# yanielc/medical-vision-textural-bias

Hardware: AMD Instinct MI355X
Metric: BraTS 4ch 240^3 vols/sec filtered+train-step @1/2/4/8 GPU; filter HBM GB/s (higher is better)
Workload: dtype f32

## Files before the change

### medical-vision-textural-bias_amd/csrc/conv_up.hip

```cpp
#include <hip/hip_runtime.h>

#include <cstdlib>
#include <type_traits>

#include "conv_host.h"
#include "split_bf16.h"
#include "texbias.h"

namespace {

typedef float f2v __attribute__((ext_vector_type(2)));
typedef float f32x4 __attribute__((ext_vector_type(4)));
typedef const __attribute__((address_space(4))) float* cfloat_p;
typedef const __attribute__((address_space(4))) f2v* cf2v_p;

template <int B, int N, class F>
__device__ __forceinline__ void static_for(F&& f) {
  if constexpr (B < N) {
    f(std::integral_constant<int, B>{});
    static_for<B + 1, N>(f);
  }
}

struct S2Args {
// ... 868 lines not shown
  for (int j = 0; j < NL; ++j) {
    const int i = tid + 256 * j;
    const int c = i / per_c, r2 = i - c * per_c, r = r2 / W4, q = r2 - r * W4;
    const int yi = y0 + r;
    lof[j] = i < total ? c * RX + r * PX + 4 * q : Wi;
    gof[j] = (i < total && yi < Hi) ? yi * Wi + 4 * q : -1;
    gch[j] = i < total ? c : 0;
  }
  float4 rg[NL];
  auto load = [&](int zi) {
    const bool in = zi < Di;
    const float* src = xb + (int64_t)(in ? zi : 0) * plane;
#pragma unroll
    for (int j = 0; j < NL; ++j) {
      const bool ok = in && gof[j] >= 0;
      rg[j] = *reinterpret_cast<const float4*>(src + gch[j] * cstride + (ok ? gof[j] : 0));
    }
  };
  auto store = [&](int zi) {
    float* d = ring + (zi & 1) * SS;
    const bool in = zi < Di;
#pragma unroll
    for (int j = 0; j < NL; ++j)
      *reinterpret_cast<float4*>(d + lof[j]) = (in && gof[j] >= 0) ? rg[j] : make_float4(0.f, 0.f, 0.f, 0.f);
  };
  float bm[4];
#pragma unroll
  for (int r = 0; r < 4; ++r) bm[r] = a.bias ? a.bias[4 * ks + r] : 0.f;
  __syncthreads();
  load(z0);
  store(z0);
  load(z0 + 1);
  store(z0 + 1);
  __builtin_amdgcn_s_waitcnt(0x0F70);
  __syncthreads();
  const int npos = YB * Wi, ntile = (npos + 15) / 16;
  const int64_t oplane = 4 * plane, orow = 2 * Wi;
  float* yb0 = a.y + (int64_t)n * 16 * (2 * Di) * oplane;
  auto sums = [&](int z, int t0, int pb) {
    const float* pr = part + pb * 4 * 8 * 256;
    for (int k = w; k < 4 * HT; k += 4) {
      const int hq = k >> 2, pz = (k >> 1) & 1, py = k & 1, q0 = pz * 4 + py * 2;
      const int pq = 16 * (t0 + hq) + li, yq = pq / Wi, xq = pq - yq * Wi;
      const bool okp = t0 + hq < ntile && pq < npos && y0 + yq < Hi;
#pragma unroll
      for (int r = 0; r < 4; ++r) {
        const int m = 4 * ks + r, e = m * 16 + li;
        float v0 = bm[r], v1 = bm[r];
#pragma unroll
        for (int v = 0; v < G; ++v) {
          v0 += pr[((hq * G + v) * 8 + q0) * 256 + e];
          v1 += pr[((hq * G + v) * 8 + q0 + 1) * 256 + e];
        }
        if (okp)
          *reinterpret_cast<float2*>(yb0 + ((int64_t)m * (2 * Di) + 2 * z + pz) * oplane +
                                     (int64_t)(2 * (y0 + yq) + py) * orow + 2 * xq) = make_float2(v0, v1);
      }
    }
  };
  int buf = 0;
  for (int z = z0; z < z1; ++z) {
    if (z + 1 < z1) load(z + 2);
    const float* sz[2] = {ring + (z & 1) * SS, ring + ((z + 1) & 1) * SS};
    for (int t0 = 0; t0 < ntile; t0 += HT) {
      const int tI = t0 + h;
      const int p = 16 * tI + li, pc = p < npos ? p : npos - 1;
      const int yy = pc / Wi, xx = pc - yy * Wi;
      const int bl = (16 * g + ks) * RX + yy * PX + xx;
      f32x4 acc[8];
#pragma unroll
      for (int q = 0; q < 8; ++q) acc[q] = f32x4{0.f, 0.f, 0.f, 0.f};
#pragma unroll
      for (int tz = 0; tz < 3; ++tz)
#pragma unroll
        for (int ty = 0; ty < 3; ++ty)
#pragma unroll
          for (int tx = 0; tx < 3; ++tx) {
            const int t = tz * 9 + ty * 3 + tx;
            const int par = (tz != 1) * 4 + (ty != 1) * 2 + (tx != 1);
            const float* s = sz[tz == 0] + bl + (ty == 0) * PX + (tx == 0);
#pragma unroll
            for (int cq = 0; cq < 4; ++cq)
              acc[par] = __builtin_amdgcn_mfma_f32_16x16x4f32(af[4 * t + cq], s[4 * cq * RX], acc[par], 0, 0, 0);
          }
      float* pw = part + (buf * 4 + w) * 8 * 256;
#pragma unroll
      for (int q = 0; q < 8; ++q)
#pragma unroll
        for (int r = 0; r < 4; ++r) pw[q * 256 + (4 * ks + r) * 16 + li] = acc[q][r];
      __syncthreads();
      if (t0 > 0) sums(z, t0 - HT, buf ^ 1);
      buf ^= 1;
    }
    store(z + 2);
    sums(z, ((ntile - 1) / HT) * HT, buf ^ 1);
    __syncthreads();
  }
}
}

int tb_convT3d_mfma64_f32(const float* x, const float* W, const float* bias, float* y, int N, int Di, int Hi, int Wi,
                          void* stream) {
  return tb_convT3d_mfma_f32(x, W, bias, y, N, 64, Di, Hi, Wi, stream);
}

int tb_convT3d_mfma_f32(const float* x, const float* W, const float* bias, float* y, int N, int Cin, int Di, int Hi,
                        int Wi, void* stream) {
  if (!x || !W || !y || N < 1 || Di < 1 || Hi < 1 || Wi < 1) return TB_ERR_INVALID_ARG;
  if (Cin != 32 && Cin != 64) return TB_ERR_UNSUPPORTED_SIZE;
  if (Wi % 4 != 0 || Wi > 64 || (reinterpret_cast<uintptr_t>(x) & 15) != 0 || (reinterpret_cast<uintptr_t>(y) & 7) != 0)
    return TB_ERR_UNSUPPORTED_SIZE;
  constexpr int YB = 2;
  T64Args a{};
  a.x = x, a.W = W, a.bias = bias, a.y = y, a.Di = Di, a.Hi = Hi, a.Wi = Wi;
  a.PX = Wi + 4;
  a.RX = (YB + 1) * a.PX;
  while ((a.RX & 31) != 16) ++a.RX;
  a.nyb = (Hi + YB - 1) / YB;
  const size_t lds = (size_t)4 * (2 * Cin * a.RX + 2 * 4 * 8 * 256);
  if (lds > 163840) return TB_ERR_UNSUPPORTED_SIZE;
  a.zlen = tb::zseg(Di, N * a.nyb, 1, 1);
  a.ZS = (Di + a.zlen - 1) / a.zlen;
  const int nl = (Cin * (YB + 1) * (Wi / 4) + 255) / 256;
  void (*kern)(T64Args) = nullptr;
  switch (nl) {
#define TB_NL(k) \
  case k: kern = Cin == 64 ? k_convT_mfma64<4, YB, k> : k_convT_mfma64<2, YB, k>; break;
    TB_NL(1) TB_NL(2) TB_NL(3) TB_NL(4) TB_NL(5) TB_NL(6) TB_NL(7) TB_NL(8) TB_NL(9) TB_NL(10) TB_NL(11) TB_NL(12)
#undef TB_NL
    default: return TB_ERR_UNSUPPORTED_SIZE;
  }
  return tb::launch_lds(kern, dim3((unsigned)(N * a.nyb * a.ZS)), dim3(256), lds,
                        reinterpret_cast<hipStream_t>(stream), a);
}

namespace {
struct S1Args {
  const float* x;
  const float* W;
  const float* bias;
  const float* add;
  float* y;
  int D, H, Wd, YB;
  int ZS, zlen, nyb, MG;
  int PX, RX;
  int flip;
  int64_t addsn;
};

template <int G, int NC, int NL, int NTH, bool ADD = false>
__global__ __launch_bounds__(NTH) void k_conv3d_mfma_s1(S1Args a) {
  constexpr int CIN = 16 * G, MTB = 4 / G, NWG = NTH / 256;
  extern __shared__ __attribute__((aligned(16))) float smem[];
  const int tid = (int)threadIdx.x, lane = tid & 63;
  const int w = __builtin_amdgcn_readfirstlane(tid >> 6);
  const int g = w % G, mt = (w / G) % MTB, h = w / 4;
  const int D = a.D, H = a.H, Wd = a.Wd, YB = a.YB, PX = a.PX, RX = a.RX, SS = CIN * RX;
  const int NR = YB + 2;
  float* ring = smem;
  float* part = smem + 3 * SS;
  float* bsm = part + (NTH / 64) * NC * 256;
  for (int i = tid; i < 3 * SS; i += NTH) ring[i] = 0.f;
  int b = (int)blockIdx.x;
  const int zs = b % a.ZS;
  b /= a.ZS;
  const int mg = b % a.MG;
  b /= a.MG;
  const int yb = b % a.nyb, n = b / a.nyb;
  const int COUT = 16 * MTB * a.MG;
  const int y0 = yb * YB;
  const int z0 = zs * a.zlen, z1 = min(D, z0 + a.zlen);
  const int li = lane & 15, ks = lane >> 4;
  const int m0 = (mg * MTB + mt) * 16;
  if (tid < MTB * 16) bsm[tid] = a.bias ? a.bias[mg * MTB * 16 + tid] : 0.f;
  float af[108];
#pragma unroll
  for (int kk = 0; kk < 108; ++kk) {
    const int c = 16 * g + 4 * (kk & 3) + ks, t = kk >> 2;
    af[kk] = a.flip ? a.W[(c * CIN + m0 + li) * 27 + 26 - t] : a.W[((m0 + li) * CIN + c) * 27 + t];
  }
  const int64_t plane = (int64_t)H * Wd, cstride = (int64_t)D * plane;
  const float* xb = a.x + (int64_t)n * CIN * cstride;
  const int W4 = Wd >> 2, per_c = NR * W4, total = CIN * per_c;
  int gof[NL], lof[NL], gch[NL];
#pragma unroll
  for (int j = 0; j < NL; ++j) {
    const int i = tid + NTH * j;
    const int c = i / per_c, r2 = i - c * per_c, r = r2 / W4, q = r2 - r * W4;
    const int yi = y0 - 1 + r;
    lof[j] = i < total ? c * RX + r * PX + 4 + 4 * q : 0;
    gof[j] = (i < total && yi >= 0 && yi < H) ? yi * Wd + 4 * q : -1;
    gch[j] = i < total ? c : 0;
  }
  float4 rg[NL];
  auto load = [&](int zi) {
    const bool in = zi >= 0 && zi < D;
    const float* src = xb + (int64_t)(in ? zi : 0) * plane;
#pragma unroll
    for (int j = 0; j < NL; ++j) {
      const bool ok = in && gof[j] >= 0;
      rg[j] = *reinterpret_cast<const float4*>(src + gch[j] * cstride + (ok ? gof[j] : 0));
    }
  };
  auto store = [&](int zi) {
    float* d = ring + ((zi + 3) % 3) * SS;
    const bool in = zi >= 0 && zi < D;
#pragma unroll
    for (int j = 0; j < NL; ++j)
      *reinterpret_cast<float4*>(d + lof[j]) = (in && gof[j] >= 0) ? rg[j] : make_float4(0.f, 0.f, 0.f, 0.f);
  };
  __syncthreads();
  load(z0 - 1);
  store(z0 - 1);
  load(z0);
  store(z0);
  load(z0 + 1);
  store(z0 + 1);
  __builtin_amdgcn_s_waitcnt(0x0F70);
  __syncthreads();
  const int npos = YB * Wd;
  float* ybase = a.y + (int64_t)n * COUT * cstride;
  const float* abase = ADD ? a.add + (int64_t)n * (a.addsn ? a.addsn : COUT * cstride) : nullptr;
  constexpr int NK = (MTB * NWG * NC + NTH / 64 - 1) / (NTH / 64);
  int bl[NC];
#pragma unroll
  for (int c = 0; c < NC; ++c) {
    const int p = 16 * (NWG * c + h) + li, pc = p < npos ? p : npos - 1;
    const int yy = pc / Wd, xx = pc - yy * Wd;
    bl[c] = (16 * g + ks) * RX + yy * PX + xx + 3;
  }
  for (int z = z0; z < z1; ++z) {
    if (z + 1 < z1) load(z + 2);
    float av[NK][4];
    if constexpr (ADD) {
#pragma unroll
      for (int kk = 0; kk < NK; ++kk) {
        const int k = w + kk * (NTH / 64);
        if (k >= MTB * NWG * NC) break;
        const int mq = k / (NWG * NC), r2 = k - mq * (NWG * NC), hq = r2 / NC, c = r2 - hq * NC;
        const int p = 16 * (NWG * c + hq) + li, pc = p < npos ? p : npos - 1;
        const int yy = pc / Wd, xx = pc - yy * Wd, yr = min(y0 + yy, H - 1);
        const int mb = (mg * MTB + mq) * 16;
#pragma unroll
        for (int r = 0; r < 4; ++r)
          av[kk][r] = abase[(int64_t)(mb + 4 * ks + r) * cstride + (int64_t)z * plane + (int64_t)yr * Wd + xx];
      }
    }
    const float* sp[3] = {ring + ((z + 2) % 3) * SS, ring + (z % 3) * SS, ring + ((z + 1) % 3) * SS};
    f32x4 acc[NC];
#pragma unroll
    for (int c = 0; c < NC; ++c) acc[c] = f32x4{0.f, 0.f, 0.f, 0.f};
#pragma unroll
    for (int tz = 0; tz < 3; ++tz)
#pragma unroll
      for (int ty = 0; ty < 3; ++ty)
#pragma unroll
        for (int tx = 0; tx < 3; ++tx) {
          const int t = tz * 9 + ty * 3 + tx;
          const float* s = sp[tz] + ty * PX + tx;
#pragma unroll
          for (int cq = 0; cq < 4; ++cq)
#pragma unroll
            for (int c = 0; c < NC; ++c)
              acc[c] = __builtin_amdgcn_mfma_f32_16x16x4f32(af[4 * t + cq], s[bl[c] + 4 * cq * RX], acc[c], 0, 0, 0);
        }
    float* pw = part + w * NC * 256;
#pragma unroll
    for (int c = 0; c < NC; ++c)
#pragma unroll
      for (int r = 0; r < 4; ++r) pw[c * 256 + (4 * ks + r) * 16 + li] = acc[c][r];
    __syncthreads();
    store(z + 2);
    auto combo = [&](int k, int kk) {
      const int mq = k / (NWG * NC), r2 = k - mq * (NWG * NC), hq = r2 / NC, c = r2 - hq * NC;
      const int p = 16 * (NWG * c + hq) + li;
      const int yy = p / Wd, xx = p - yy * Wd;
      const bool ok = p < npos && y0 + yy < H;
      const int mb = (mg * MTB + mq) * 16;
#pragma unroll
      for (int r = 0; r < 4; ++r) {
        const int m = 4 * ks + r;
        float v = bsm[mq * 16 + m];
#pragma unroll
        for (int gg = 0; gg < G; ++gg) v += part[((hq * 4 + mq * G + gg) * NC + c) * 256 + m * 16 + li];
        const int64_t o = (int64_t)(mb + m) * cstride + (int64_t)z * plane + (int64_t)(y0 + yy) * Wd + xx;
        if (ok) ybase[o] = ADD ? v + av[kk][r] : v;
      }
    };
    if constexpr (ADD) {
#pragma unroll
      for (int kk = 0; kk < NK; ++kk) {
        const int k = w + kk * (NTH / 64);
        if (k >= MTB * NWG * NC) break;
        combo(k, kk);
      }
    } else {
      for (int k = w; k < MTB * NWG * NC; k += NTH / 64) combo(k, 0);
    }
    __syncthreads();
  }
}
}

int tb_conv3d_mfma_f32(const float* x, const float* W, const float* bias, float* y, int N, int C, int D, int H, int Wd,
                       void* stream) {
  return tb_conv3d_mfma_add_f32(x, W, bias, nullptr, y, N, C, D, H, Wd, stream);
}

static int mfma_call(const float* x, const float* W, const float* bias, const float* add, float* y, int N, int C, int D,
                     int H, int Wd, int flip, void* stream, int64_t add_sn = 0);

int tb_conv3d_mfma_add_f32(const float* x, const float* W, const float* bias, const float* add, float* y, int N, int C,
                           int D, int H, int Wd, void* stream) {
  return mfma_call(x, W, bias, add, y, N, C, D, H, Wd, 0, stream);
}

int tb_conv3d_mfma_dgrad_f32(const float* gy, const float* W, const float* add, int64_t add_sn, float* dx, int N, int C,
                             int D, int H, int Wd, void* stream) {
  return mfma_call(gy, W, nullptr, add, dx, N, C, D, H, Wd, 1, stream, add_sn);
}

static int mfma_call(const float* x, const float* W, const float* bias, const float* add, float* y, int N, int C, int D,
                     int H, int Wd, int flip, void* stream, int64_t add_sn) {
  if (!x || !W || !y || N < 1 || D < 1 || H < 1 || Wd < 1) return TB_ERR_INVALID_ARG;
  if ((C != 32 && C != 64) || Wd % 4 != 0 || Wd > 64 || (reinterpret_cast<uintptr_t>(x) & 15) != 0)
    return TB_ERR_UNSUPPORTED_SIZE;
  constexpr int NC = 5;
  const int G = C / 16;
  S1Args a{};
  a.x = x, a.W = W, a.bias = bias, a.add = add, a.y = y, a.D = D, a.H = H, a.Wd = Wd;
  a.flip = flip;
  a.addsn = add_sn;
  a.PX = Wd + 8;
  a.MG = G == 2 ? 1 : 4;
  size_t lds = 0;
  int YB = std::max(1, 16 * NC / Wd);
  for (; YB >= 1; --YB) {
    a.RX = (YB + 2) * a.PX;
    while ((a.RX & 31) != 16) ++a.RX;
    lds = (size_t)4 * (3 * C * a.RX + 4 * NC * 256 + 64);
    if (lds <= 163840) break;
  }
  if (YB < 1) return TB_ERR_UNSUPPORTED_SIZE;
  a.YB = YB > H ? H : YB;
  a.nyb = (H + a.YB - 1) / a.YB;
  a.zlen = tb::zseg(D, N * a.nyb * a.MG, 1, 2);
  a.ZS = (D + a.zlen - 1) / a.zlen;
  const int nl = (C * (a.YB + 2) * (Wd / 4) + 255) / 256;
  void (*kern)(S1Args) = nullptr;
#define TB_NL(k)                                                                                      \
  case k:                                                                                             \
    kern = add ? (G == 2 ? k_conv3d_mfma_s1<2, 5, k, 256, true> : k_conv3d_mfma_s1<4, 5, k, 256, true>) \
               : (G == 2 ? k_conv3d_mfma_s1<2, 5, k, 256> : k_conv3d_mfma_s1<4, 5, k, 256>);             \
    break;
  switch (nl) {
    TB_NL(1) TB_NL(2) TB_NL(3) TB_NL(4) TB_NL(5) TB_NL(6) TB_NL(7) TB_NL(8) TB_NL(9) TB_NL(10) TB_NL(11) TB_NL(12)
    default: return TB_ERR_UNSUPPORTED_SIZE;
  }
#undef TB_NL
  return tb::launch_lds(kern, dim3((unsigned)(N * a.nyb * a.MG * a.ZS)), dim3(256), lds,
                        reinterpret_cast<hipStream_t>(stream), a);
}
```

Before: 186.1.

## Add z-streaming split-bf16 MFMA conv kernel with register-resident weights and LDS ring

Adds a new 3D conv kernel for C=32/64 that keeps the split-bf16 weight fragments in registers and streams input z-planes through a 3-slot LDS ring. Input planes are pre-split into three bf16 parts when stored, with the next plane prefetched into registers during compute. Partial sums from the channel groups are reduced through LDS before bias/add and the store. It becomes the default path whenever the plan fits, trading higher register pressure and extra LDS synchronisation for less global reload of the input halo and less per-tap conversion work.

```diff
diff --git a/medical-vision-textural-bias_amd/csrc/conv_up.hip b/medical-vision-textural-bias_amd/csrc/conv_up.hip
--- a/medical-vision-textural-bias_amd/csrc/conv_up.hip
+++ b/medical-vision-textural-bias_amd/csrc/conv_up.hip
@@ -1194,6 +1194,179 @@
 }
 }
 
+namespace {
+struct XSArgs {
+  const float* x;
+  const float* W;
+  const float* bias;
+  const float* add;
+  float* y;
+  int D, H, Wd, YB;
+  int ZS, zlen, nyb, MG;
+  int ntile;
+  int flip;
+  int64_t addsn;
+};
+
+inline size_t xs_slot(int G, int YB, int W) { return (size_t)3 * G * (YB + 2) * (W + 5) * 32; }
+
+template <int G, int MTB, bool ADD>
+__global__ __launch_bounds__(512) void k_conv_mfma_split(XSArgs a) {
+  using tb::bf16x8;
+  constexpr int CIN = 16 * G, NTH = 512, NWV = NTH / 64, NROLE = G * MTB, NWG = NWV / NROLE;
+  static_assert(NROLE * NWG == NWV, "every wave has a role");
+  extern __shared__ __attribute__((aligned(16))) char ringx[];
+  const int tid = (int)threadIdx.x, lane = tid & 63;
+  const int w = __builtin_amdgcn_readfirstlane(tid >> 6);
+  const int grp = w % G, mt = (w / G) % MTB, h = w / NROLE;
+  const int D = a.D, H = a.H, Wd = a.Wd, YB = a.YB, NR = YB + 2;
+  const int RPB = (Wd + 5) * 32, GPB = NR * RPB, SPL = G * GPB, SLOT = 3 * SPL;
+  char* part = ringx + 3 * SLOT;
+  float* bsm = reinterpret_cast<float*>(part + a.ntile * NROLE * 1024);
+  for (int i = tid; i < 3 * SLOT / 16; i += NTH) reinterpret_cast<uint4*>(ringx)[i] = make_uint4(0, 0, 0, 0);
+  int b = (int)blockIdx.x;
+  const int zs = b % a.ZS;
+  b /= a.ZS;
+  const int mg = b % a.MG;
+  b /= a.MG;
+  const int yb = b % a.nyb, n = b / a.nyb;
+  const int COUT = 16 * MTB * a.MG;
+  const int y0 = yb * YB;
+  const int z0 = zs * a.zlen, z1 = min(D, z0 + a.zlen);
+  if (tid < MTB * 16) bsm[tid] = a.bias ? a.bias[mg * MTB * 16 + tid] : 0.f;
+  const int li = lane & 15, g4 = lane >> 4, hi = g4 >> 1;
+  const int m0 = (mg * MTB + mt) * 16;
+  bf16x8 af[14][3];
+  {
+    const int wsm = a.flip ? 27 : CIN * 27, wsc = a.flip ? CIN * 27 : 27;
+    const float* wl = a.W + (m0 + li) * wsm + (16 * grp + 8 * (g4 & 1)) * wsc;
+#pragma unroll
+    for (int q = 0; q < 14; ++q) {
+      const int t = 2 * q + hi, tc = t < 27 ? t : 26;
+      const float* wq = wl + (a.flip ? 26 - tc : tc);
+      float v[8];
+#pragma unroll
+      for (int j = 0; j < 8; ++j) v[j] = wq[j * wsc];
+      if (q == 13) {
+#pragma unroll
+        for (int j = 0; j < 8; ++j) v[j] = hi ? 0.f : v[j];
+      }
+      tb::split3(v, af[q][0], af[q][1], af[q][2]);
+    }
+  }
+  const int64_t plane = (int64_t)H * Wd, cstride = (int64_t)D * plane;
+  const char* xb = reinterpret_cast<const char*>(a.x + (int64_t)n * CIN * cstride);
+  const int W4 = Wd >> 2;
+  const int cq = tid & 3, rr = (tid >> 2) % NR, r2 = (tid >> 2) / NR, q4 = r2 % W4, sg = r2 / W4;
+  const bool act = sg < G;
+  const int lof = act ? sg * GPB + rr * RPB + (4 * q4 + 1) * 32 + cq * 8 : (Wd + 1) * 32;
+  const int yi = y0 - 1 + rr;
+  const bool rowok = act && yi >= 0 && yi < H;
+  const unsigned chb = (unsigned)(4 * cstride);
+  const unsigned gof = rowok ? (unsigned)(16 * sg + 4 * cq) * chb + 4u * (unsigned)(yi * Wd + 4 * q4) : 0u;
+  float4 rg[4];
+  auto load = [&](int zi) {
+    const char* src = xb + (int64_t)(zi < 0 ? 0 : zi >= D ? D - 1 : zi) * plane * 4;
+#pragma unroll
+    for (int c = 0; c < 4; ++c) rg[c] = *reinterpret_cast<const float4*>(src + c * chb + gof);
+  };
+  auto store = [&](int zi) {
+    char* d = ringx + ((zi + 3) % 3) * SLOT + lof;
+    const unsigned m = 0u - (unsigned)(rowok && zi >= 0 && zi < D);
+#pragma unroll
+    for (int e = 0; e < 4; ++e) {
+      float v[4];
+#pragma unroll
+      for (int c = 0; c < 4; ++c)
+        v[c] = __uint_as_float(__float_as_uint(e == 0 ? rg[c].x : e == 1 ? rg[c].y : e == 2 ? rg[c].z : rg[c].w) & m);
+      unsigned p[3][2];
+      tb::split3_pk(v[0], v[1], p[0][0], p[1][0], p[2][0]);
+      tb::split3_pk(v[2], v[3], p[0][1], p[1][1], p[2][1]);
+#pragma unroll
+      for (int s = 0; s < 3; ++s) *reinterpret_cast<uint2*>(d + s * SPL + e * 32) = make_uint2(p[s][0], p[s][1]);
+    }
+  };
+  __syncthreads();
+  load(z0 - 1);
+  store(z0 - 1);
+  load(z0);
+  store(z0);
+  load(z0 + 1);
+  store(z0 + 1);
+  __builtin_amdgcn_s_waitcnt(0x0F70);
+  __syncthreads();
+  const int npos = YB * Wd, ntile = a.ntile;
+  float* ybase = a.y + (int64_t)n * COUT * cstride;
+  const float* abase = ADD ? a.add + (int64_t)n * (a.addsn ? a.addsn : COUT * cstride) : nullptr;
+  const int lb = grp * GPB + 16 * (g4 & 1);
+  for (int z = z0; z < z1; ++z) {
+    load(z + 2);
+    int hv = hi;
+    asm volatile("" : "+v"(hv));
+    int sb[3];
+#pragma unroll
+    for (int tz = 0; tz < 3; ++tz) sb[tz] = ((z + tz + 2) % 3) * SLOT;
+    for (int t = h; t < ntile; t += NWG) {
+      const int p = 16 * t + li, pc = p < npos ? p : npos - 1;
+      const int yy = pc / Wd, xx = pc - yy * Wd;
+      const char* rb = ringx + lb + yy * RPB + xx * 32;
+      bf16x8 bq[2][3];
+      auto ldb = [&](int q, bf16x8 (&bf)[3]) {
+        const int t0 = 2 * q, t1 = 2 * q + 1 < 27 ? 2 * q + 1 : 26;
+        const int c0 = sb[t0 / 9] + ((t0 / 3) % 3) * RPB + (t0 % 3) * 32;
+        const int c1 = sb[t1 / 9] + ((t1 / 3) % 3) * RPB + (t1 % 3) * 32;
+        const int o = hv ? c1 : c0;
+        bf[1] = *reinterpret_cast<const bf16x8*>(rb + o + SPL);
+        bf[2] = *reinterpret_cast<const bf16x8*>(rb + o + 2 * SPL);
+        bf[0] = *reinterpret_cast<const bf16x8*>(rb + o);
+      };
+      tb::f32x4s c = {0.f, 0.f, 0.f, 0.f}, cs = c;
+      ldb(0, bq[0]);
+#pragma unroll
+      for (int q = 0; q < 14; ++q) {
+        if (q + 1 < 14) ldb(q + 1, bq[(q + 1) & 1]);
+        tb::mfma_split6(af[q], bq[q & 1], c, cs);
+      }
+      c += cs;
+      __builtin_amdgcn_sched_group_barrier(0x100, 3, 0);
+#pragma unroll
+      for (int q = 0; q < 13; ++q) {
+        __builtin_amdgcn_sched_group_barrier(0x100, 3, 0);
+        __builtin_amdgcn_sched_group_barrier(0x008, 6, 0);
+      }
+      __builtin_amdgcn_sched_group_barrier(0x008, 6, 0);
+      *reinterpret_cast<tb::f32x4s*>(part + ((t * NROLE + mt * G + grp) * 64 + lane) * 16) = c;
+    }
+    __syncthreads();
+    store(z + 2);
+    for (int k = w; k < ntile * MTB; k += NWV) {
+      const int t = k / MTB, mq = k - t * MTB;
+      const int p = 16 * t + li, pc = p < npos ? p : npos - 1;
+      const int yy = pc / Wd, xx = pc - yy * Wd;
+      const bool ok = p < npos && y0 + yy < H;
+      const int mb = (mg * MTB + mq) * 16 + 4 * g4;
+      const unsigned oo = (unsigned)(mb * cstride + (int64_t)min(y0 + yy, H - 1) * Wd + xx);
+      float av[4];
+      if constexpr (ADD) {
+#pragma unroll
+        for (int r = 0; r < 4; ++r) av[r] = (abase + (int64_t)z * plane)[oo + (unsigned)r * (unsigned)cstride];
+      }
+      const char* pr = part + ((t * NROLE + mq * G) * 64 + lane) * 16;
+      tb::f32x4s v = *reinterpret_cast<const tb::f32x4s*>(pr);
+#pragma unroll
+      for (int gg = 1; gg < G; ++gg) v += *reinterpret_cast<const tb::f32x4s*>(pr + gg * 1024);
+#pragma unroll
+      for (int r = 0; r < 4; ++r) {
+        float o = v[r] + bsm[mq * 16 + 4 * g4 + r];
+        if constexpr (ADD) o += av[r];
+        if (ok) (ybase + (int64_t)z * plane)[oo + (unsigned)r * (unsigned)cstride] = o;
+      }
+    }
+    __syncthreads();
+  }
+}
+}
+
 int tb_conv3d_mfma_f32(const float* x, const float* W, const float* bias, float* y, int N, int C, int D, int H, int Wd,
                        void* stream) {
   return tb_conv3d_mfma_add_f32(x, W, bias, nullptr, y, N, C, D, H, Wd, stream);
@@ -1210,6 +1383,21 @@
 int tb_conv3d_mfma_dgrad_f32(const float* gy, const float* W, const float* add, int64_t add_sn, float* dx, int N, int C,
                              int D, int H, int Wd, void* stream) {
   return mfma_call(gy, W, nullptr, add, dx, N, C, D, H, Wd, 1, stream, add_sn);
+}
+
+static bool xs_plan(int C, int D, int H, int Wd, XSArgs& s, size_t& lds) {
+  if ((int64_t)C * D * H * Wd >= (1LL << 29) || (C == 32 && Wd < 16)) return false;
+  const int G = C / 16, MTB = G == 2 ? 2 : 1;
+  for (int YB = std::min(4, H); YB >= 1; --YB) {
+    const int ntile = (YB * Wd + 15) / 16;
+    lds = 3 * xs_slot(G, YB, Wd) + (size_t)ntile * G * MTB * 1024 + MTB * 64;
+    if (4 * G * (YB + 2) * (Wd / 4) > 512 || lds > 163840) continue;
+    s.D = D, s.H = H, s.Wd = Wd, s.YB = YB, s.ntile = ntile;
+    s.nyb = (H + YB - 1) / YB;
+    s.MG = C / (16 * MTB);
+    return true;
+  }
+  return false;
 }
 
 static int mfma_call(const float* x, const float* W, const float* bias, const float* add, float* y, int N, int C, int D,
@@ -1217,6 +1405,19 @@
   if (!x || !W || !y || N < 1 || D < 1 || H < 1 || Wd < 1) return TB_ERR_INVALID_ARG;
   if ((C != 32 && C != 64) || Wd % 4 != 0 || Wd > 64 || (reinterpret_cast<uintptr_t>(x) & 15) != 0)
     return TB_ERR_UNSUPPORTED_SIZE;
+  {
+    XSArgs s{};
+    size_t slds = 0;
+    if (xs_plan(C, D, H, Wd, s, slds)) {
+      s.x = x, s.W = W, s.bias = bias, s.add = add, s.y = y, s.flip = flip, s.addsn = add_sn;
+      s.zlen = tb::zseg(D, N * s.nyb * s.MG, 1, 2);
+      s.ZS = (D + s.zlen - 1) / s.zlen;
+      void (*sk)(XSArgs) = C == 32 ? (add ? k_conv_mfma_split<2, 2, true> : k_conv_mfma_split<2, 2, false>)
+                                   : (add ? k_conv_mfma_split<4, 1, true> : k_conv_mfma_split<4, 1, false>);
+      return tb::launch_lds(sk, dim3((unsigned)(N * s.nyb * s.MG * s.ZS)), dim3(512), slds,
+                            reinterpret_cast<hipStream_t>(stream), s);
+    }
+  }
   constexpr int NC = 5;
   const int G = C / 16;
   S1Args a{};
```

Result: faster. 194.3, median of 6 (+4.4%).
